# rlorenzo/facet

Measured on AMD Instinct MI355X. Metric: images/sec whole-node (TOPIQ+SAMP+CLIP+InsightFace ensemble), 1024² batch, higher is better.
Workload: dtype f32

## Files before the change

### facet_amd/csrc/engine.hip

```cpp
#include "engine.h"
#include "onnx_graph.h"
#include <algorithm>
#include <cmath>
#include <cstdlib>

namespace fe {

void WeightStore::set(const std::string& name, const float* data, const int64_t* shape, int ndim) {
  HostTensor h;
  h.shape.assign(shape, shape + ndim);
  h.data.assign(data, data + h.numel());
  t_[name] = std::move(h);
}
const HostTensor& WeightStore::get(const std::string& name) const {
  auto it = t_.find(name);
  if (it == t_.end()) throw Error("missing weight tensor '" + name + "'");
  return it->second;
}

float* DeviceWeights::upload(const std::vector<float>& v) {
  void* p = nullptr;
  const size_t b = v.size() * sizeof(float);
  FE_HIP(hipMalloc(&p, b ? b : 16));
  if (b) FE_HIP(hipMemcpy(p, v.data(), b, hipMemcpyHostToDevice));
  ptrs_.push_back(p);
  bytes_ += b;
  return (float*)p;
}
void* DeviceWeights::upload_raw(const void* data, size_t bytes) {
  void* p = nullptr;
  FE_HIP(hipMalloc(&p, bytes ? bytes : 16));
  if (bytes) FE_HIP(hipMemcpy(p, data, bytes, hipMemcpyHostToDevice));
  ptrs_.push_back(p);
  bytes_ += bytes;
  return p;
}
void DeviceWeights::release() {
  for (void* p : ptrs_) (void)hipFree(p);
  ptrs_.clear();
  bytes_ = 0;
}

const float* to_f32(Ctx& c, const bf16* p, size_t n) {
  float* f = c.arena.array<float>(n);
  launch_convert(p, f, n, c.stream);
  return f;
}
const float* to_f32(Ctx& c, const f16* p, size_t n) {
  float* f = c.arena.array<float>(n);
  launch_convert(p, f, n, c.stream);
  return f;
}

Ctx::~Ctx() {
  topiq.reset();
  for (auto& kv : resize_box_cache) { (void)hipFree(kv.second.kk); (void)hipFree(kv.second.bounds); }
  for (auto& kv : jpeg_cache) (void)hipFree(kv.second);
  if (jpegdec_stage) (void)hipHostFree(jpegdec_stage);
  arena.release();
  if (stream) (void)hipStreamDestroy(stream);
}

ConvW pack_conv(DeviceWeights& dw, const HostTensor& w, const std::vector<float>* scale, const std::vector<float>* shift) {
  FE_CHECK(w.shape.size() == 4 || w.shape.size() == 2, "conv weight rank %zu", w.shape.size());
  ConvW c;
  c.Cout = (int)w.shape[0];
  c.Cin = (int)w.shape[1];
  c.KH = w.shape.size() == 4 ? (int)w.shape[2] : 1;
  c.KW = w.shape.size() == 4 ? (int)w.shape[3] : 1;
  c.CinPad = (c.Cin + 3) & ~3;
  c.K = c.KH * c.KW * c.CinPad;
  c.Kp = (c.K + CONV_KALIGN - 1) / CONV_KALIGN * CONV_KALIGN;
  std::vector<float> packed((size_t)c.Cout * c.Kp, 0.f);
  const bool blocked = (c.CinPad % 16 == 0);
  const int ntaps = c.KH * c.KW;
  for (int co = 0; co < c.Cout; ++co)
    for (int ci = 0; ci < c.Cin; ++ci)
      for (int kh = 0; kh < c.KH; ++kh)
        for (int kw = 0; kw < c.KW; ++kw) {
          const int tap = kh * c.KW + kw;
          const size_t k = blocked ? ((size_t)(ci / 16) * ntaps + tap) * 16 + (ci % 16) : (size_t)tap * c.CinPad + ci;
          packed[(size_t)co * c.Kp + k] = w.data[(((size_t)co * c.Cin + ci) * c.KH + kh) * c.KW + kw];
        }
  const bool skip_f32 = dw.half_only && dw.prec != PREC_F32 && (c.KH * c.KW == 1 || ((c.Cin + 7) & ~7) % 16 == 0);
  if (!skip_f32) c.w = dw.upload(packed);
  if (!skip_f32 && c.Cout <= 2 && c.KH * c.KW > 1 && c.CinPad % 16 == 0) {
    const int T = c.KH * c.KW * c.Cout;
    c.KpT = (c.CinPad + CONV_KALIGN - 1) / CONV_KALIGN * CONV_KALIGN;
    std::vector<float> tp((size_t)T * c.KpT, 0.f);
    for (int t = 0; t < c.KH * c.KW; ++t)
      for (int co = 0; co < c.Cout; ++co)
        for (int ci = 0; ci < c.Cin; ++ci)
          tp[(size_t)(t * c.Cout + co) * c.KpT + ci] = w.data[(((size_t)co * c.Cin + ci) * c.KH + t / c.KW) * c.KW + t % c.KW];
    c.wtap = dw.upload(tp);
  }
  if (c.CinPad == 4 && c.KH == c.KW && (c.KH == 7 || c.KH == 3) && (c.Cout == 32 || c.Cout == 64)) {
    bool ch3_zero = true;
    const int taps = c.KH * c.KW, taps2 = (taps + 1) & ~1;
    for (int co = 0; co < c.Cout && c.Cin == 4; ++co)
      for (int t = 0; t < taps; ++t) ch3_zero = ch3_zero && w.data[((size_t)co * c.Cin + 3) * taps + t] == 0.f;
    if (ch3_zero) {
      std::vector<float> st((size_t)taps2 * c.Cout * 4, 0.f);
      for (int co = 0; co < c.Cout; ++co)
        for (int ci = 0; ci < c.Cin && ci < 3; ++ci)
          for (int t = 0; t < taps; ++t) st[((size_t)t * c.Cout + co) * 4 + ci] = w.data[((size_t)co * c.Cin + ci) * taps + t];
      c.wstem = dw.upload(st);
    }
  }
  static const int wino_min_cin = getenv("FE_WINO_MIN_CIN") ? atoi(getenv("FE_WINO_MIN_CIN")) : 96;
  static const int wino_form = getenv("FE_WINO_FORM") ? atoi(getenv("FE_WINO_FORM")) : 4;
  if (!skip_f32 && dw.prec == PREC_F32 && (wino_form == 2 || wino_form == 4) && c.KH == 3 && c.KW == 3 && c.Cin == c.CinPad && c.Cin % 32 == 0 && c.Cin >= wino_min_cin && c.Cout % 4 == 0) {
    static const double G2[4][3] = {{1, 0, 0}, {0.5, 0.5, 0.5}, {0.5, -0.5, 0.5}, {0, 0, 1}};
    static const double G4[6][3] = {{0.25, 0, 0}, {-1.0 / 6, -1.0 / 6, -1.0 / 6}, {-1.0 / 6, 1.0 / 6, -1.0 / 6},
                                    {1.0 / 24, 1.0 / 12, 1.0 / 6}, {1.0 / 24, -1.0 / 12, 1.0 / 6}, {0, 0, 1}};
    const int R = wino_form == 2 ? 4 : 6;
    auto Gm = [&](int a, int q) { return wino_form == 2 ? G2[a][q] : G4[a][q]; };
    std::vector<float> U((size_t)R * R * c.Cout * c.Cin);
    for (int co = 0; co < c.Cout; ++co)
      for (int ci = 0; ci < c.Cin; ++ci) {
        const float* g = &w.data[((size_t)co * c.Cin + ci) * 9];
        double tmp[6][3];
        for (int a = 0; a < R; ++a)
          for (int q = 0; q < 3; ++q) tmp[a][q] = Gm(a, 0) * g[q] + Gm(a, 1) * g[3 + q] + Gm(a, 2) * g[6 + q];
        for (int a = 0; a < R; ++a)
          for (int b = 0; b < R; ++b) {
            const double u = tmp[a][0] * Gm(b, 0) + tmp[a][1] * Gm(b, 1) + tmp[a][2] * Gm(b, 2);
            U[((size_t)(R * a + b) * c.Cout + co) * c.Cin + ci] = (float)u;
          }
      }
    c.wino = dw.upload(U);
    c.wino_m = wino_form;
  }
  if (scale) c.scale = dw.upload(*scale);
  if (shift) c.shift = dw.upload(*shift);
  if (dw.prec != PREC_F32) pack_conv_bf16(dw, w, c);
  return c;
}

void pack_conv_bf16(DeviceWeights& dw, const HostTensor& w, ConvW& c) {
  const int ntaps = c.KH * c.KW;
  c.CinPadH = (c.Cin + 7) & ~7;
  if (ntaps > 1) {
    if (c.CinPadH % 32 == 0) c.cb = 32;
    else if (c.CinPadH % 16 == 0) c.cb = 16;
    else return;
    if (ntaps >= 64) return;
  } else {
    c.cb = 32;
  }
  const int K = ntaps * c.CinPadH;
  c.KpH = (K + CONV_KALIGN_H - 1) / CONV_KALIGN_H * CONV_KALIGN_H;
  std::vector<uint16_t> packed((size_t)c.Cout * c.KpH, 0);
  for (int co = 0; co < c.Cout; ++co)
    for (int ci = 0; ci < c.Cin; ++ci)
      for (int t = 0; t < ntaps; ++t) {
        const size_t k = ntaps > 1 ? ((size_t)(ci / c.cb) * ntaps + t) * c.cb + (ci % c.cb) : (size_t)ci;
        packed[(size_t)co * c.KpH + k] = f32_to_half_bits(w.data[((size_t)co * c.Cin + ci) * ntaps + t], dw.prec);
      }
  c.wh = dw.upload_raw(packed.data(), packed.size() * sizeof(uint16_t));
  c.hprec = dw.prec;
  if (c.Cout <= 2 && ntaps > 1) {
    const int T = ntaps * c.Cout, T8 = (T + 7) & ~7;
    c.KpTH = (c.CinPadH + CONV_KALIGN_H - 1) / CONV_KALIGN_H * CONV_KALIGN_H;
    std::vector<uint16_t> tp((size_t)T8 * c.KpTH, 0);
    for (int t = 0; t < ntaps; ++t)
      for (int co = 0; co < c.Cout; ++co)
        for (int ci = 0; ci < c.Cin; ++ci)
          tp[(size_t)(t * c.Cout + co) * c.KpTH + ci] = f32_to_half_bits(w.data[((size_t)co * c.Cin + ci) * ntaps + t], dw.prec);
    c.wtap_h = dw.upload_raw(tp.data(), tp.size() * sizeof(uint16_t));
  }
}

ConvW build_conv(DeviceWeights& dw, const WeightStore& ws, const std::string& conv_prefix,
                 const std::string& bn_prefix, bool conv_bias, float bn_eps) {
  const HostTensor& w = ws.get(conv_prefix + ".weight");
  const int cout = (int)w.shape[0];
  std::vector<float> scale, shift;
  const bool bn = !bn_prefix.empty();
  if (bn) {
    const auto& g = ws.get(bn_prefix + ".weight").data;
    const auto& b = ws.get(bn_prefix + ".bias").data;
    const auto& mu = ws.get(bn_prefix + ".running_mean").data;
    const auto& var = ws.get(bn_prefix + ".running_var").data;
    FE_CHECK((int)g.size() == cout && (int)var.size() == cout, "bn %s size mismatch", bn_prefix.c_str());
    scale.resize(cout); shift.resize(cout);
    for (int i = 0; i < cout; ++i) {
      const float inv = 1.0f / std::sqrt(var[i] + bn_eps);
      scale[i] = g[i] * inv;
      float sh = b[i] - mu[i] * scale[i];
      if (conv_bias) sh += ws.get(conv_prefix + ".bias").data[i] * scale[i];
      shift[i] = sh;
    }
  } else if (conv_bias) {
    shift = ws.get(conv_prefix + ".bias").data;
    FE_CHECK((int)shift.size() == cout, "bias %s size mismatch", conv_prefix.c_str());
  }
  return pack_conv(dw, w, scale.empty() ? nullptr : &scale, shift.empty() ? nullptr : &shift);
}

ConvW build_linear(DeviceWeights& dw, const WeightStore& ws, const std::string& prefix, bool bias) {
  const HostTensor& w = ws.get(prefix + ".weight");
  FE_CHECK(w.shape.size() == 2, "linear %s weight rank", prefix.c_str());
  if (bias) {
    const auto& b = ws.get(prefix + ".bias").data;
    return pack_conv(dw, w, nullptr, &b);
  }
  return pack_conv(dw, w, nullptr, nullptr);
}

ConvW build_linear_rows(DeviceWeights& dw, const HostTensor& w, const HostTensor* b, int row0, int rows) {
  FE_CHECK(w.shape.size() == 2 && row0 + rows <= w.shape[0], "linear_rows: bad range");
  HostTensor sub;
  const int in = (int)w.shape[1];
  sub.shape = {rows, in};
// ... 22 lines not shown
  p.x = x.p; p.ldx = x.ld;
  p.w = w.w; p.scale = w.scale; p.shift = w.shift; p.slope = w.slope;
  FE_CHECK(o.act != ACT_PRELU || w.slope, "conv: PReLU without slopes");
  if (o.res) {
    FE_CHECK(o.res->c == y.c && o.res->pixels() == y.pixels(), "conv: residual shape mismatch");
    p.res = o.res->p; p.ldr = o.res->ld;
  }
  if (o.gate) {
    FE_CHECK(o.gate->pixels() == y.pixels() && (o.gate->c == 1 || o.gate->c == y.c), "conv: gate shape mismatch");
    p.gate = o.gate->p; p.ldg = o.gate->ld; p.gate_c1 = o.gate->c == 1;
  }
  p.y = y.p; p.ldy = y.ld;
  p.N = x.n; p.H = x.h; p.W = x.w; p.Cin = w.CinPad;
  p.Ho = y.h; p.Wo = y.w; p.Cout = w.Cout;
  p.KH = w.KH; p.KW = w.KW; p.sh = o.sh; p.sw = o.sw; p.ph = o.ph; p.pw = o.pw; p.dh = o.dh; p.dw = o.dw;
  FE_CHECK(y.h == conv_out_dim(x.h, w.KH, o.sh, o.ph, o.dh) && y.w == conv_out_dim(x.w, w.KW, o.sw, o.pw, o.dw),
           "conv: output dims %dx%d inconsistent with input %dx%d", y.h, y.w, x.h, x.w);
  p.K = w.K; p.Kp = w.Kp;
  p.M = (int)y.pixels();
  FE_CHECK(y.pixels() < (1ull << 31), "conv: M too large");
  p.act = o.act; p.res_after_act = o.res_after_act;
  p.variant = c.force_variant;
  if (w.wtap && o.act != ACT_PRELU && o.sh == 1 && o.sw == 1 && !o.res && !o.gate && p.variant == 0 && y.h == x.h && y.w == x.w) {
    const int T = w.KH * w.KW * w.Cout, Tp = (T + 3) & ~3;
    const size_t mark = c.arena.mark();
    Tensor z = c.arena.tensor(x.n, x.h, x.w, Tp);
    ConvParams q{};
    q.x = x.p; q.ldx = x.ld; q.w = w.wtap; q.y = z.p; q.ldy = Tp;
    q.N = x.n; q.H = x.h; q.W = x.w; q.Cin = w.CinPad; q.Ho = x.h; q.Wo = x.w; q.Cout = T;
    q.KH = q.KW = 1; q.sh = q.sw = q.dh = q.dw = 1;
    q.K = w.CinPad; q.Kp = w.KpT; q.M = (int)x.pixels();
    launch_conv(q, c.stream);
    launch_tap_gather(z.p, Tp, x.n, x.h, x.w, w.KH, w.KW, o.ph, o.pw, o.dh, o.dw, w.Cout, w.scale, w.shift, o.act, y.p,
                      y.ld, y.h, y.w, c.stream);
    c.arena.rewind(mark);
    c.flops_accum += 2.0 * p.M * (double)(w.KH * w.KW * w.Cin) * (w.CoutAlg ? w.CoutAlg : p.Cout);
    return;
  }
  static const bool no_wino = getenv("FE_NO_WINO") != nullptr;
  const bool wino_plain = !o.res && (o.act == ACT_NONE || o.act == ACT_RELU);
  if (w.wino && !no_wino && p.variant == 0 && o.sh == 1 && o.sw == 1 && o.ph == 1 && o.pw == 1 && o.dh == 1 && o.dw == 1 &&
      !o.gate && (wino_plain || (w.wino_m == 4 && (o.act == ACT_NONE || o.act == ACT_RELU || o.act == ACT_PRELU))) && y.h == x.h && y.w == x.w && (((uintptr_t)x.p | (uintptr_t)y.p) & 15) == 0 &&
      x.ld % 4 == 0 && y.ld % 4 == 0) {
    const int ts = w.wino_m, planes = (ts + 2) * (ts + 2);
    const int th = (x.h + ts - 1) / ts, tw = (x.w + ts - 1) / ts;
    const size_t tiles = (size_t)x.n * th * tw;
    const size_t wino_bytes = (size_t)planes * tiles * ((size_t)w.CinPad + w.Cout) * sizeof(float) + 1024;
    if (tiles < (1u << 30) / 36 && c.arena.mark() + wino_bytes <= c.arena.capacity()) {
      const size_t mark = c.arena.mark();
      float* V = (float*)c.arena.alloc((size_t)planes * tiles * w.CinPad * sizeof(float));
      float* Mb = (float*)c.arena.alloc((size_t)planes * tiles * w.Cout * sizeof(float));
      hipEvent_t e0 = nullptr, e1 = nullptr;
      if (c.profile) {
        FE_HIP(hipEventCreate(&e0)); FE_HIP(hipEventCreate(&e1));
        FE_HIP(hipEventRecord(e0, c.stream));
      }
      if (ts == 2) launch_wino_input(x, th, tw, V, c.stream);
      else launch_wino4_input(x, th, tw, V, c.stream);
      ConvParams g{};
      g.x = V; g.ldx = w.CinPad; g.w = w.wino; g.ldw = w.CinPad; g.y = Mb; g.ldy = w.Cout;
      g.M = (int)tiles; g.K = w.CinPad; g.Cout = w.Cout;
      g.N = 1; g.H = 1; g.W = g.M; g.Ho = 1; g.Wo = g.M; g.KH = g.KW = 1; g.sh = g.sw = g.dh = g.dw = 1;
      g.Kp = w.CinPad; g.Cin = w.CinPad;
      g.batch = planes; g.nb1 = 1; g.xs2 = (long long)tiles * w.CinPad; g.ws2 = (long long)w.Cout * w.CinPad; g.ys2 = (long long)tiles * w.Cout;
      launch_conv(g, c.stream);
      if (ts == 2) launch_wino_output(Mb, y, th, tw, w.scale, w.shift, o.act == ACT_RELU, c.stream);
      else launch_wino4_output(Mb, y, th, tw, w.scale, w.shift, o.act, w.slope, o.res, o.res_after_act, c.stream);
      if (c.profile) {
        FE_HIP(hipEventRecord(e1, c.stream));
        FE_HIP(hipEventSynchronize(e1));
        float ms = 0.f;
        FE_HIP(hipEventElapsedTime(&ms, e0, e1));
        (void)hipEventDestroy(e0); (void)hipEventDestroy(e1);
        char nm[128];
        snprintf(nm, sizeof nm, "wino3x3 M=%d K=%d N=%d", p.M, p.K, p.Cout);
        c.timings.push_back({nm, 2.0 * p.M * (double)(9 * w.Cin) * p.Cout, 0.0, ms});
      }
      c.arena.rewind(mark);
      c.flops_accum += 2.0 * p.M * (double)(w.KH * w.KW * w.Cin) * (w.CoutAlg ? w.CoutAlg : p.Cout);
      c.flops_saved += 2.0 * p.M * (double)(9 * w.Cin) * (w.CoutAlg ? w.CoutAlg : p.Cout) - 2.0 * (double)planes * (double)tiles * w.CinPad * w.Cout;
      return;
    }
  }
  static const bool no_splitk = getenv("FE_NO_SPLITK") != nullptr;
  if (!no_splitk && w.KH == 1 && w.KW == 1 && o.sh == 1 && o.sw == 1 && o.ph == 0 && o.pw == 0 && !o.gate && p.variant == 0 && p.M <= 256 &&
      w.CinPad >= (getenv("FE_SPLITK_MIN") ? atoi(getenv("FE_SPLITK_MIN")) : 2048) && w.K == w.CinPad &&
      (o.act == ACT_NONE || o.act == ACT_RELU || o.act == ACT_PRELU)) {
    int splits = 0;
    for (int s = 64; s >= 2; --s)
      if (w.CinPad % s == 0 && (w.CinPad / s) % 32 == 0 && w.CinPad / s >= 256) { splits = s; break; }
    const size_t part_bytes = (size_t)splits * p.M * w.Cout * sizeof(float);
    if (splits && c.arena.mark() + part_bytes + 1024 <= c.arena.capacity()) {
      const size_t mark = c.arena.mark();
      float* part = (float*)c.arena.alloc(part_bytes);
      const int Ks = w.CinPad / splits;
      hipEvent_t e0 = nullptr, e1 = nullptr;
      if (c.profile) {
        FE_HIP(hipEventCreate(&e0)); FE_HIP(hipEventCreate(&e1));
        FE_HIP(hipEventRecord(e0, c.stream));
      }
      ConvParams g{};
      g.x = x.p; g.ldx = x.ld; g.w = w.w; g.ldw = w.Kp; g.y = part; g.ldy = w.Cout;
      g.M = p.M; g.K = Ks; g.Kp = Ks; g.Cin = Ks; g.Cout = w.Cout;
      g.N = 1; g.H = 1; g.W = g.M; g.Ho = 1; g.Wo = g.M; g.KH = g.KW = 1; g.sh = g.sw = g.dh = g.dw = 1;
      g.batch = splits; g.nb1 = 1; g.xs2 = Ks; g.ws2 = Ks; g.ys2 = (long long)p.M * w.Cout;
      launch_conv(g, c.stream);
      launch_splitk_reduce(part, splits, p.M, w.Cout, w.scale, w.shift, w.slope, o.act, o.res ? o.res->p : nullptr, o.res ? o.res->ld : 0,
                           o.res_after_act, y.p, y.ld, c.stream);
      if (c.profile) {
        FE_HIP(hipEventRecord(e1, c.stream));
        FE_HIP(hipEventSynchronize(e1));
        float ms = 0.f;
        FE_HIP(hipEventElapsedTime(&ms, e0, e1));
        (void)hipEventDestroy(e0); (void)hipEventDestroy(e1);
        char nm[128];
        snprintf(nm, sizeof nm, "splitk%d 1x1 M=%d K=%d N=%d", splits, p.M, p.K, p.Cout);
        c.timings.push_back({nm, 2.0 * p.M * (double)w.Cin * (w.CoutAlg ? w.CoutAlg : p.Cout), 0.0, ms});
      }
      c.arena.rewind(mark);
      c.flops_accum += 2.0 * p.M * (double)w.Cin * (w.CoutAlg ? w.CoutAlg : p.Cout);
      return;
    }
  }
  static const bool no_stem = getenv("FE_NO_STEM") != nullptr;
  const bool stem = w.wstem && !no_stem && p.variant == 0 && o.sh == o.sw && o.ph == w.KH / 2 && o.pw == w.KW / 2 && o.dh == 1 && o.dw == 1 && !o.res &&
                    !o.gate && (o.act == ACT_NONE || o.act == ACT_RELU || o.act == ACT_PRELU);
  auto launch = [&]() {
    if (stem && launch_stem(x.p, x.ld, x.n, x.h, x.w, w.wstem, w.scale, w.shift, w.slope, w.Cout, w.KH, o.sh,
                            o.act == ACT_RELU ? 1 : (o.act == ACT_PRELU ? 2 : 0), y.p, y.ld, y.h, y.w, c.stream))
      return;
    launch_conv(p, c.stream);
  };
  if (c.profile) {
    hipEvent_t e0, e1;
    FE_HIP(hipEventCreate(&e0)); FE_HIP(hipEventCreate(&e1));
    FE_HIP(hipEventRecord(e0, c.stream));
    launch();
    FE_HIP(hipEventRecord(e1, c.stream));
    FE_HIP(hipEventSynchronize(e1));
    float ms = 0.f;
    FE_HIP(hipEventElapsedTime(&ms, e0, e1));
    (void)hipEventDestroy(e0); (void)hipEventDestroy(e1);
    char nm[128];
    snprintf(nm, sizeof nm, "conv%dx%d s%d d%d M=%d K=%d N=%d", w.KH, w.KW, o.sh, o.dh, p.M, p.K, p.Cout);
    double bytes = 4.0 * ((double)x.pixels() * x.c + (double)y.pixels() * y.c * (o.res ? 2 : 1) + (double)w.Cout * w.K);
    c.timings.push_back({nm, 2.0 * p.M * (double)(w.KH * w.KW * w.Cin) * (w.CoutAlg ? w.CoutAlg : p.Cout), bytes, ms});
  } else {
    launch();
  }
  c.flops_accum += 2.0 * p.M * (double)(w.KH * w.KW * w.Cin) * (w.CoutAlg ? w.CoutAlg : p.Cout);
}

template <class E>
static void conv_forward_half(Ctx& c, const ConvW& w, const TensorT<E>& x, const TensorT<E>& y, const ConvOptsT<E>& o) {
  if (!w.wh && w.w && PrecOf<E>::value != PREC_F32 && !o.res && !o.gate && x.ld == x.c && y.ld == y.c && x.c >= w.CinPad) {
    const size_t mark = c.arena.mark();
    Tensor xf = c.arena.tensor(x.n, x.h, x.w, x.c), yf = c.arena.tensor(y.n, y.h, y.w, y.c);
    launch_convert(x.p, xf.p, x.numel(), c.stream);
    ConvOpts of; of.sh = o.sh; of.sw = o.sw; of.ph = o.ph; of.pw = o.pw; of.dh = o.dh; of.dw = o.dw; of.act = o.act;
    conv_forward(c, w, xf.slice(0, w.CinPad), yf, of);
    launch_convert(yf.p, y.p, y.numel(), c.stream);
    c.arena.rewind(mark);
    return;
  }
  FE_CHECK(w.wh && w.hprec == PrecOf<E>::value, "conv(2-byte): this layer has no weights of the activations' type (model committed under another "
           "precision, or a 3-channel first layer)");
  FE_CHECK(x.c == w.CinPadH, "conv(bf16): input channels %d != packed Cin %d", x.c, w.CinPadH);
  FE_CHECK(y.c == w.Cout && y.n == x.n, "conv(bf16): output view mismatch (c=%d Cout=%d)", y.c, w.Cout);
  FE_CHECK(y.p || o.y32, "conv(2-byte): no output tensor");
// ... 448 lines not shown
```

### facet_amd/csrc/fe_common.h

```cpp
#pragma once
#include <hip/hip_runtime.h>
#include "fe_check.h"
#include <cstdint>
#include <cstdio>
#include <atomic>
#include <cstring>
#include <map>
#include <mutex>
#include <stdexcept>
#include <string>
#include <vector>

namespace fe {


#define FE_HIP(expr)                                                                      \
  do {                                                                                    \
    hipError_t _e = (expr);                                                               \
    if (_e != hipSuccess) {                                                               \
      char _b[512];                                                                       \
      snprintf(_b, sizeof _b, "%s:%d: %s -> %s", __FILE__, __LINE__, #expr,               \
               hipGetErrorString(_e));                                                    \
      throw fe::Error(_b);                                                                \
    }                                                                                     \
// ... 141 lines not shown
    FE_HIP(hipMalloc(&base_, bytes));
    cap_ = bytes;
    off_ = 0;
  }
  void release() {
    if (base_) (void)hipFree(base_);
    base_ = nullptr;
    cap_ = off_ = 0;
  }
  ~Arena() { release(); }
  void reset() { off_ = 0; }
  size_t mark() const { return off_; }
  void rewind(size_t m) { off_ = m; }
  size_t capacity() const { return cap_; }
  size_t high_water() const { return high_; }
  void* alloc(size_t bytes) {
    size_t a = (off_ + 255) & ~(size_t)255;
    FE_CHECK(a + bytes <= cap_, "arena exhausted: need %zu at %zu of %zu", bytes, a, cap_);
    off_ = a + bytes;
    if (off_ > high_) high_ = off_;
    return (char*)base_ + a;
  }
  template <class T>
  TensorT<T> tensor_t(int n, int h, int w, int c) {
    TensorT<T> t;
    t.n = n; t.h = h; t.w = w; t.c = c; t.ld = c;
    t.p = (T*)alloc(t.numel() * sizeof(T));
    return t;
  }
  Tensor tensor(int n, int h, int w, int c) { return tensor_t<float>(n, h, w, c); }
  template <class T>
  T* array(size_t count) { return (T*)alloc(count * sizeof(T)); }
 private:
  void* base_ = nullptr;
  size_t cap_ = 0, off_ = 0, high_ = 0;
};

template <class T>
struct ConvParamsT {
  const T* x; int ldx;
  const T* w;
  const float* scale;
  const float* shift;
  const float* slope;
  const T* res; int ldr;
  const T* gate; int ldg;
  T* y; int ldy;
  int N, H, W, Cin, Ho, Wo, Cout;
  int KH, KW, sh, sw, ph, pw, dh, dw;
  int K, Kp, M;
  int act;
  int res_after_act;
  int gate_c1;
  int vec_epi;
  int unit_stride;
  int ldw;
  int batch, nb1;
  long long xs1, xs2, ws1, ws2, ys1, ys2, hs1;
  int buf_ok; unsigned x_span, w_span;
  unsigned y_span, r_span, g_span;
  int variant;
  int cb;
  int pad_store;
  const float* res32; int ldr32;
  float* y32; int ldy32;
  unsigned r32_span, y32_span;
  int a_wrap;
  int split_lo_off;
  int exact_act;
};
using ConvParams = ConvParamsT<float>;
using ConvParamsH = ConvParamsT<bf16>;

struct ConvW {
  float* w = nullptr;
  float* scale = nullptr;
  float* shift = nullptr;
  float* slope = nullptr;
  int Cout = 0, Cin = 0, CinPad = 0, KH = 1, KW = 1, K = 0, Kp = 0;
  int CoutAlg = 0;
  float* wtap = nullptr;
  int wino_m = 0;
  float* wino = nullptr;
  float* wstem = nullptr;
  float* wn16 = nullptr;
  int KpT = 0;
  void* wh = nullptr;
  int hprec = 0;
  int KpH = 0, cb = 0, CinPadH = 0;
  void* wtap_h = nullptr;
  int KpTH = 0;
  uint8_t* w8 = nullptr;
  float* w8_scale = nullptr;
};

template <class T>
struct ConvOptsT {
  int sh = 1, sw = 1, ph = 0, pw = 0, dh = 1, dw = 1;
  int act = ACT_NONE;
  const TensorT<T>* res = nullptr;
  int res_after_act = 0;
  const TensorT<T>* gate = nullptr;
  const TensorT<float>* res32 = nullptr;
  const TensorT<float>* y32 = nullptr;
};
using ConvOpts = ConvOptsT<float>;

constexpr int CONV_KALIGN = 32;
constexpr int CONV_KALIGN_H = 64;

void launch_conv(const ConvParams& p, hipStream_t s);
void launch_wino_input(const Tensor& x, int th, int tw, float* V, hipStream_t s);
void launch_wino_output(const float* Mb, const Tensor& y, int th, int tw, const float* scale, const float* shift, int relu, hipStream_t s);
void launch_wino4_input(const Tensor& x, int th, int tw, float* V, hipStream_t s);
void launch_wino4_output(const float* Mb, const Tensor& y, int th, int tw, const float* scale, const float* shift, int act, const float* slope,
                         const Tensor* res, int res_after_act, hipStream_t s);
template <class TO>
bool launch_stem(const float* x, int ldx, int N, int H, int W, const float* wstem, const float* scale, const float* shift, const float* slope,
                 int Cout, int k, int stride, int act, TO* y, int ldy, int Ho, int Wo, hipStream_t s);
void launch_conv_narrow(const ConvParams& p, hipStream_t s);
void launch_conv_dma(const ConvParams& p, int tile, hipStream_t s);
void launch_conv_bf16(const ConvParamsH& p, hipStream_t s);
void launch_conv_bf16(const ConvParamsT<f16>& p, hipStream_t s);
template <class T, class Launch>
inline bool conv_split_by_images(const ConvParamsT<T>& p, Launch&& launch) {
  if (p.batch > 1 || p.N <= 1 || (long long)p.N * p.Ho * p.Wo != (long long)p.M) return false;
  const unsigned long long in_img = (unsigned long long)p.H * p.W * p.ldx * sizeof(T);
  unsigned long long out_img = (unsigned long long)p.Ho * p.Wo * (unsigned long long)(p.ldy > p.ldr ? p.ldy : p.ldr) * sizeof(T);
  const unsigned long long out32_img = (unsigned long long)p.Ho * p.Wo * (unsigned long long)(p.ldy32 > p.ldr32 ? p.ldy32 : p.ldr32) * sizeof(float);
  if ((p.y32 || p.res32) && out32_img > out_img) out_img = out32_img;
  const unsigned long long per_img = in_img > out_img ? in_img : out_img;
  constexpr unsigned long long LIMIT = 0xF0000000ull;
  if (per_img >= LIMIT) return false;
  const int ng = (int)(LIMIT / per_img);
  if (ng >= p.N) return false;
  for (int i0 = 0; i0 < p.N; i0 += ng) {
    ConvParamsT<T> q = p;
    const int n = ng < p.N - i0 ? ng : p.N - i0;
    const size_t opix = (size_t)i0 * p.Ho * p.Wo;
    q.N = n; q.M = n * p.Ho * p.Wo;
    q.x = p.x + (size_t)i0 * p.H * p.W * p.ldx;
    if (p.y) q.y = p.y + opix * p.ldy;
    if (p.y32) q.y32 = p.y32 + opix * p.ldy32;
    if (p.res32) q.res32 = p.res32 + opix * p.ldr32;
    if (p.res) q.res = p.res + opix * p.ldr;
    if (p.gate) q.gate = p.gate + opix * p.ldg;
    launch(q);
  }
  return true;
}

double conv_flops(const ConvParams& p);

void launch_u8_to_nhwc4_norm(const uint8_t* src, float* dst, size_t pixels, const float mean[3],
                             const float stdv[3], int bgr, hipStream_t s);
template <class T> void launch_nchw_to_nhwc(const float* src, T* dst, int n, int c, int h, int w, int cpad, hipStream_t s);
template <class T> void launch_nhwc_to_nchw(const T* src, int lds_, float* dst, int n, int c, int h, int w, hipStream_t s);
template <class T> void launch_maxpool(const TensorT<T>& x, const TensorT<T>& y, int k, int stride, int pad, hipStream_t s);
template <class T> void launch_bilinear(const TensorT<T>& x, const TensorT<T>& y, hipStream_t s);
template <class T> void launch_adaptive_avgpool(const TensorT<T>& x, const TensorT<T>& y, hipStream_t s);
void launch_convert(const float* x, bf16* y, size_t n, hipStream_t s);
void launch_convert(const bf16* x, float* y, size_t n, hipStream_t s);
void launch_convert(const float* x, f16* y, size_t n, hipStream_t s);
void launch_convert(const f16* x, float* y, size_t n, hipStream_t s);
void launch_splitk_reduce(const float* part, int splits, int M, int N, const float* scale, const float* shift, const float* slope, int act,
                          const float* res, int ldr, int res_after_act, float* y, int ldy, hipStream_t s);
template <class T>
void launch_tap_gather(const T* z, int ldz, int n, int h, int w, int kh, int kw, int ph, int pw, int dh, int dw,
                       int cout, const float* scale, const float* shift, int act, T* y, int ldy, int ho, int wo,
                       hipStream_t s);
void launch_attention(const float* q, int ldq, const float* k, int ldk, const float* vt, int lp, const float* bv, float* o,
                      int ldo, int B, int H, int Lq, int Lk, int dmodel, int causal, hipStream_t s);
void launch_attention(const bf16* q, int ldq, const bf16* k, int ldk, const bf16* vt, int lp, const float* bv, bf16* o,
                      int ldo, int B, int H, int Lq, int Lk, int dmodel, int causal, hipStream_t s);
void launch_attention(const f16* q, int ldq, const f16* k, int ldk, const f16* vt, int lp, const float* bv, f16* o,
                      int ldo, int B, int H, int Lq, int Lk, int dmodel, int causal, hipStream_t s);
void launch_attention_split(const f16* q, const f16* k, int ld, int lo_off, const f16* vt_hi, const f16* vt_lo, int lp, f16* o, int ldo, int o_lo_off,
                            int B, int H, int Lq, int Lk, int dmodel, hipStream_t s);
template <class TI, class TW, class TO>
void launch_gemm_skinny(const TI* x, int ldx, const TW* w, int ldw, const float* scale, const float* shift, TO* y,
                        int ldy, int M, int N, int K, int act, hipStream_t s);
void launch_sigmoid(const Tensor& x, const Tensor& y, hipStream_t s);
void launch_add(const Tensor& a, const Tensor& b, const Tensor& y, hipStream_t s);
void launch_layernorm_split(const float* x, int ldx, f16* y, int ldy, const float* g, const float* b, int rows, int d, float eps, hipStream_t s);
void launch_split_hi_lo(const float* x, f16* y, size_t rows, int cols, hipStream_t s);
template <class T, class TO>
void launch_layernorm(const T* x, int ldx, TO* y, int ldy, const float* g, const float* b,
                      int rows, int d, float eps, hipStream_t s);
void launch_softmax_rows(float* x, int ld, int rows, int d, hipStream_t s);
void launch_softmax_rows_pad(float* x, int ld, int rows, int d, hipStream_t s);
template <class T>
void launch_add_rows_bcast(T* y, int ldy, const float* pos, int rows, int L, int d, hipStream_t s);

void launch_affine_act(const Tensor& x, const Tensor& y, const float* scale, const float* shift, int act, const float* slope,
                       hipStream_t s);
void launch_binary(const Tensor& a, const Tensor& b, const Tensor& y, int op, int act, hipStream_t s);
void launch_gather_strided(const float* src, float* dst, const long long dims[6], const long long sstr[6], hipStream_t s);
void launch_nearest(const Tensor& x, const Tensor& y, hipStream_t s);
void launch_avgpool(const Tensor& x, const Tensor& y, int k, int stride, int pad, int include_pad, hipStream_t s);
// ... 49 lines not shown
```

Baseline: 231.4.

## Add fused Winograd F(2x2,3x3) MFMA kernel for 64-channel 3x3 convs

Adds a single-kernel Winograd F(2,3) path for stride-1, pad-1 3x3 convolutions with 56-64 input and 33-64 output channels. It stages input patches through double-buffered LDS, does the input transform in registers, runs the per-plane products on 32x32x2 f32 MFMA, and applies the output transform, affine, activation and residual in the epilogue. This replaces the separate input-transform, GEMM and output-transform launches and their intermediate buffers. It also restricts split-K for 1x1 convs to small tile grids and caches the split-K threshold environment variable. The added cost is a new, complex kernel with one block per CU and a 2x2 Winograd form that saves less arithmetic than F(4,3).

```diff
diff --git a/facet_amd/csrc/engine.hip b/facet_amd/csrc/engine.hip
--- a/facet_amd/csrc/engine.hip
+++ b/facet_amd/csrc/engine.hip
@@ -1,5 +1,6 @@
 #include "engine.h"
 #include "onnx_graph.h"
+#include "wino64_maps.h"
 #include <algorithm>
 #include <cmath>
 #include <cstdlib>
@@ -130,6 +131,11 @@
       }
     c.wino = dw.upload(U);
     c.wino_m = wino_form;
+  }
+  if (!skip_f32 && dw.prec == PREC_F32 && c.KH == 3 && c.KW == 3 && c.CinPad >= 56 && c.CinPad <= 64 && c.Cout > 32 && c.Cout <= 64 && c.Cout % 4 == 0) {
+    std::vector<float> U(w64::U_FLOATS);
+    w64::pack_u(w.data.data(), c.Cout, c.Cin, U.data());
+    c.wino64 = dw.upload(U);
   }
   if (scale) c.scale = dw.upload(*scale);
   if (shift) c.shift = dw.upload(*shift);
@@ -318,9 +324,37 @@
       return;
     }
   }
+  static const bool no_wino64 = getenv("FE_NO_WINO64") != nullptr;
+  if (w.wino64 && !no_wino64 && p.variant == 0 && (o.act == ACT_NONE || o.act == ACT_RELU || o.act == ACT_PRELU) && o.sh == 1 && o.sw == 1 && o.ph == 1 && o.pw == 1 && o.dh == 1 && o.dw == 1 && !o.gate && y.h == x.h &&
+      y.w == x.w && (((uintptr_t)x.p | (uintptr_t)y.p | (uintptr_t)(o.res ? o.res->p : nullptr)) & 15) == 0 && x.ld % 4 == 0 && y.ld % 4 == 0 &&
+      (!o.res || o.res->ld % 4 == 0) && (unsigned long long)x.h * x.w * x.ld * 4ull < 0xF0000000ull) {
+    hipEvent_t e0 = nullptr, e1 = nullptr;
+    if (c.profile) {
+      FE_HIP(hipEventCreate(&e0)); FE_HIP(hipEventCreate(&e1));
+      FE_HIP(hipEventRecord(e0, c.stream));
+    }
+    launch_wino64(x, y, w.wino64, w.scale, w.shift, w.slope, o.act, o.res, o.res_after_act, c.stream);
+    const double direct = 2.0 * p.M * (double)(9 * w.Cin) * (w.CoutAlg ? w.CoutAlg : p.Cout);
+    if (c.profile) {
+      FE_HIP(hipEventRecord(e1, c.stream));
+      FE_HIP(hipEventSynchronize(e1));
+      float ms = 0.f;
+      FE_HIP(hipEventElapsedTime(&ms, e0, e1));
+      (void)hipEventDestroy(e0); (void)hipEventDestroy(e1);
+      char nm[128];
+      snprintf(nm, sizeof nm, "wino64 3x3 M=%d K=%d N=%d", p.M, p.K, p.Cout);
+      const double bytes = 4.0 * ((double)x.pixels() * x.c + (double)y.pixels() * y.c * (o.res ? 2 : 1) + (double)w64::U_FLOATS);
+      c.timings.push_back({nm, direct, bytes, ms});
+    }
+    const double tiles = (double)x.n * ((x.h + 1) / 2) * ((x.w + 1) / 2);
+    c.flops_accum += direct;
+    c.flops_saved += direct - 2.0 * 16.0 * tiles * 64.0 * w.Cout;
+    return;
+  }
   static const bool no_splitk = getenv("FE_NO_SPLITK") != nullptr;
+  static const int splitk_min = getenv("FE_SPLITK_MIN") ? atoi(getenv("FE_SPLITK_MIN")) : 2048;
   if (!no_splitk && w.KH == 1 && w.KW == 1 && o.sh == 1 && o.sw == 1 && o.ph == 0 && o.pw == 0 && !o.gate && p.variant == 0 && p.M <= 256 &&
-      w.CinPad >= (getenv("FE_SPLITK_MIN") ? atoi(getenv("FE_SPLITK_MIN")) : 2048) && w.K == w.CinPad &&
+      w.CinPad >= splitk_min && w.K == w.CinPad && (size_t)((p.M + 127) / 128) * ((w.Cout + 63) / 64) < 64 &&
       (o.act == ACT_NONE || o.act == ACT_RELU || o.act == ACT_PRELU)) {
     int splits = 0;
     for (int s = 64; s >= 2; --s)
diff --git a/facet_amd/csrc/fe_common.h b/facet_amd/csrc/fe_common.h
--- a/facet_amd/csrc/fe_common.h
+++ b/facet_amd/csrc/fe_common.h
@@ -247,6 +247,7 @@
   float* wtap = nullptr;
   int wino_m = 0;
   float* wino = nullptr;
+  float* wino64 = nullptr;
   float* wstem = nullptr;
   float* wn16 = nullptr;
   int KpT = 0;
@@ -280,6 +281,8 @@
 void launch_wino4_input(const Tensor& x, int th, int tw, float* V, hipStream_t s);
 void launch_wino4_output(const float* Mb, const Tensor& y, int th, int tw, const float* scale, const float* shift, int act, const float* slope,
                          const Tensor* res, int res_after_act, hipStream_t s);
+void launch_wino64(const Tensor& x, const Tensor& y, const float* U, const float* scale, const float* shift, const float* slope, int act,
+                   const Tensor* res, int res_after_act, hipStream_t s);
 template <class TO>
 bool launch_stem(const float* x, int ldx, int N, int H, int W, const float* wstem, const float* scale, const float* shift, const float* slope,
                  int Cout, int k, int stride, int act, TO* y, int ldy, int Ho, int Wo, hipStream_t s);
diff --git a/facet_amd/csrc/kernels_wino64.hip b/facet_amd/csrc/kernels_wino64.hip
--- /dev/null
+++ b/facet_amd/csrc/kernels_wino64.hip
@@ -0,0 +1,205 @@
+#include "fe_common.h"
+#include "wino64_maps.h"
+
+namespace fe {
+
+struct W64Params {
+  const float* x; int ldx, cin;
+  int N, H, W;
+  float* y; int ldy, cout;
+  const float* U;
+  const float *scale, *shift, *slope;
+  const float* res; int ldr;
+  int res_after_act;
+  int bx, by, nblocks;
+};
+
+constexpr int W64_PATCH_FLOATS = w64::CHUNK_UNITS * 2;
+
+template <int A>
+__global__ __launch_bounds__(256, 1) __attribute__((amdgpu_waves_per_eu(1, 1))) void wino64_kernel(const W64Params p) {
+  using namespace w64;
+  __shared__ __attribute__((aligned(16))) float sP[2 * W64_PATCH_FLOATS];
+  const int t = threadIdx.x, lane = t & 63, wave = __builtin_amdgcn_readfirstlane(t >> 6);
+  const int tg = wave & 1, half = wave >> 1;
+  const int tl = lane & 31, kk = lane >> 5;
+  const int ty = tile_y(tg, tl), tx = tile_x(tl);
+  constexpr int act = A;
+
+  int pc_py[PIECES_PER_THREAD], pc_px[PIECES_PER_THREAD], pc_dst[PIECES_PER_THREAD];
+#pragma unroll
+  for (int i = 0; i < PIECES_PER_THREAD; ++i) {
+    const int idx = t + 256 * i, pixel = idx / PARTS, part = idx % PARTS;
+    pc_py[i] = pixel / PATCH; pc_px[i] = pixel - pc_py[i] * PATCH;
+    pc_dst[i] = idx < PIECES ? 2 * patch_unit(2 * part, pc_py[i], pc_px[i]) : -1;
+  }
+  const int part4 = (t % PARTS) * 4;
+  auto block_origin = [&](const int v, int& b, int& y0, int& x0) {
+    const int per = p.bx * p.by;
+    b = v / per;
+    const int rem = v - b * per, byi = rem / p.bx;
+    y0 = byi * BLOCK; x0 = (rem - byi * p.bx) * BLOCK;
+  };
+  fe_v4f pf[PIECES_PER_THREAD];
+  typedef unsigned w64_v4u __attribute__((ext_vector_type(4)));
+  constexpr unsigned OOB = 0xFFFFFFF0u;
+  const unsigned img_bytes = (unsigned)p.H * (unsigned)p.W * (unsigned)p.ldx * 4u;
+  auto fetch_stage = [&](const int v, const int c) __attribute__((always_inline)) {
+    const bool live = v < p.nblocks;
+    int b, y0, x0;
+    block_origin(live ? v : 0, b, y0, x0);
+    const __amdgpu_buffer_rsrc_t rs = __builtin_amdgcn_make_buffer_rsrc(const_cast<float*>(p.x + (size_t)b * p.H * p.W * p.ldx), 0, (int)img_bytes, 0x00020000);
+    const bool ch_in = live && c * CHUNK_CH + part4 < p.cin;
+#pragma unroll
+    for (int i = 0; i < PIECES_PER_THREAD; ++i) {
+      const int gy = y0 - 1 + pc_py[i], gx = x0 - 1 + pc_px[i];
+      const bool in = pc_dst[i] >= 0 && ch_in && (unsigned)gy < (unsigned)p.H && (unsigned)gx < (unsigned)p.W;
+      const unsigned off = in ? ((unsigned)(gy * p.W + gx) * (unsigned)p.ldx + (unsigned)(c * CHUNK_CH + part4)) * 4u : OOB;
+      pf[i] = __builtin_bit_cast(fe_v4f, (w64_v4u)__builtin_amdgcn_raw_buffer_load_b128(rs, (int)off, 0, 0));
+    }
+  };
+  auto store_stage = [&](const int buf) __attribute__((always_inline)) {
+    float* const pd = sP + buf * W64_PATCH_FLOATS;
+#pragma unroll
+    for (int i = 0; i < PIECES_PER_THREAD; ++i)
+      if (pc_dst[i] >= 0) {
+        *reinterpret_cast<float2*>(pd + pc_dst[i]) = make_float2(pf[i].x, pf[i].y);
+        *reinterpret_cast<float2*>(pd + pc_dst[i] + 2 * PAIR_UNITS) = make_float2(pf[i].z, pf[i].w);
+      }
+  };
+
+  const float* const ubase = p.U + u_index(0, half, 0, lane, 0);
+  fe_v4f ua[STEPS_PER_CHUNK][4];
+  auto fetch_u = [&](const int step, fe_v4f (&u)[4]) __attribute__((always_inline)) {
+#pragma unroll
+    for (int q = 0; q < 4; ++q) u[q] = *reinterpret_cast<const fe_v4f*>(ubase + step * U_STEP_FLOATS + q * 256);
+  };
+#pragma unroll
+  for (int s0 = 0; s0 < STEPS_PER_CHUNK; ++s0) fetch_u(s0, ua[s0]);
+  fetch_stage(blockIdx.x, 0);
+  store_stage(0);
+  __syncthreads();
+
+  const int lane_unit = patch_unit(kk, 2 * ty, 2 * tx);
+  for (int v = blockIdx.x; v < p.nblocks; v += gridDim.x) {
+    fe_f32x16 acc[16];
+#pragma unroll
+    for (int pl = 0; pl < 16; ++pl)
+#pragma unroll
+      for (int e = 0; e < 16; ++e) acc[pl][e] = 0.f;
+
+#pragma unroll 1
+    for (int c = 0; c < NCHUNK; ++c) {
+      if (c + 1 < NCHUNK) fetch_stage(v, c + 1);
+      else fetch_stage(v + (int)gridDim.x, 0);
+      const float* const buf = sP + (c & 1) * W64_PATCH_FLOATS + 2 * lane_unit;
+      float2 dq[2][16];
+      auto read_pair = [&](const int j, float2 (&d)[16]) __attribute__((always_inline)) {
+#pragma unroll
+        for (int dy = 0; dy < 4; ++dy)
+#pragma unroll
+          for (int dx = 0; dx < 4; ++dx)
+            d[4 * dy + dx] = *reinterpret_cast<const float2*>(buf + 2 * (2 * j * PAIR_UNITS + dy * ROW_UNITS + (dx & 1) * (ROW_UNITS / 2) + (dx >> 1)));
+      };
+      const int nstage = ((c + 1) & (NCHUNK - 1)) * STEPS_PER_CHUNK;
+      read_pair(0, dq[0]);
+#pragma unroll
+      for (int j = 0; j < STEPS_PER_CHUNK / 2; ++j) {
+        if (j + 1 < STEPS_PER_CHUNK / 2) read_pair(j + 1, dq[(j + 1) & 1]);
+        __builtin_amdgcn_sched_barrier(0);
+#pragma unroll
+        for (int s2 = 0; s2 < 2; ++s2) {
+          float d[16], vv[16];
+#pragma unroll
+          for (int i = 0; i < 16; ++i) d[i] = s2 ? dq[j & 1][i].y : dq[j & 1][i].x;
+          input_transform(d, vv);
+#pragma unroll
+          for (int pl = 0; pl < 16; ++pl) acc[pl] = __builtin_amdgcn_mfma_f32_32x32x2f32(ua[2 * j + s2][pl >> 2][pl & 3], vv[pl], acc[pl], 0, 0, 0);
+          __builtin_amdgcn_sched_barrier(0);
+          fetch_u(nstage + 2 * j + s2, ua[2 * j + s2]);
+        }
+      }
+      store_stage((c + 1) & 1);
+      __syncthreads();
+    }
+
+    int b, y0, x0;
+    block_origin(v, b, y0, x0);
+    const int oy = y0 + 2 * ty, ox = x0 + 2 * tx;
+    size_t pix[4]; bool ok[4];
+#pragma unroll
+    for (int i = 0; i < 4; ++i) {
+      const int yy = oy + (i >> 1), xx = ox + (i & 1);
+      ok[i] = yy < p.H && xx < p.W;
+      pix[i] = ok[i] ? ((size_t)b * p.H + yy) * p.W + xx : 0;
+    }
+    float4 scv[4], sfv[4], slv[4];
+#pragma unroll
+    for (int g = 0; g < 4; ++g) {
+      const int cb = acc_channel(half, lane, 4 * g), cl = cb < p.cout ? cb : 0;
+      scv[g] = p.scale ? *reinterpret_cast<const float4*>(p.scale + cl) : make_float4(1.f, 1.f, 1.f, 1.f);
+      sfv[g] = p.shift ? *reinterpret_cast<const float4*>(p.shift + cl) : make_float4(0.f, 0.f, 0.f, 0.f);
+      slv[g] = act == ACT_PRELU ? *reinterpret_cast<const float4*>(p.slope + cl) : make_float4(0.f, 0.f, 0.f, 0.f);
+    }
+#pragma unroll
+    for (int g = 0; g < 4; ++g) {
+      const int cb = acc_channel(half, lane, 4 * g);
+      if (cb >= p.cout) continue;
+      float o[4][4];
+#pragma unroll
+      for (int e = 0; e < 4; ++e) {
+        float m[16], yq[4];
+#pragma unroll
+        for (int pl = 0; pl < 16; ++pl) m[pl] = acc[pl][4 * g + e];
+        output_transform(m, yq);
+#pragma unroll
+        for (int i = 0; i < 4; ++i) o[i][e] = yq[i];
+      }
+      const float4 sc = scv[g], sf = sfv[g], sl = slv[g];
+#pragma unroll
+      for (int i = 0; i < 4; ++i) {
+        if (!ok[i]) continue;
+        float4 r = make_float4(0.f, 0.f, 0.f, 0.f);
+        if (p.res) r = *reinterpret_cast<const float4*>(p.res + pix[i] * p.ldr + cb);
+        float4 q;
+        q.x = o[i][0] * sc.x + sf.x; q.y = o[i][1] * sc.y + sf.y; q.z = o[i][2] * sc.z + sf.z; q.w = o[i][3] * sc.w + sf.w;
+        if (p.res && !p.res_after_act) { q.x += r.x; q.y += r.y; q.z += r.z; q.w += r.w; }
+        if (act == ACT_PRELU) {
+          q.x = q.x > 0.f ? q.x : q.x * sl.x; q.y = q.y > 0.f ? q.y : q.y * sl.y;
+          q.z = q.z > 0.f ? q.z : q.z * sl.z; q.w = q.w > 0.f ? q.w : q.w * sl.w;
+        } else {
+          q.x = fe_apply_act(q.x, act); q.y = fe_apply_act(q.y, act); q.z = fe_apply_act(q.z, act); q.w = fe_apply_act(q.w, act);
+        }
+        if (p.res && p.res_after_act) { q.x += r.x; q.y += r.y; q.z += r.z; q.w += r.w; }
+        *reinterpret_cast<float4*>(p.y + pix[i] * p.ldy + cb) = q;
+      }
+    }
+  }
+}
+
+void launch_wino64(const Tensor& x, const Tensor& y, const float* U, const float* scale, const float* shift, const float* slope, int act,
+                   const Tensor* res, int res_after_act, hipStream_t s) {
+  FE_CHECK(x.c > 0 && x.c <= 64 && x.c % 4 == 0 && y.c > 0 && y.c <= 64 && y.c % 4 == 0 && y.n == x.n && y.h == x.h && y.w == x.w, "wino64: %dx%dx%d -> %dx%dx%d", x.h,
+           x.w, x.c, y.h, y.w, y.c);
+  FE_CHECK(x.ld % 4 == 0 && y.ld % 4 == 0 && (((uintptr_t)x.p | (uintptr_t)y.p | (uintptr_t)U) & 15) == 0, "wino64: operands must be 16-byte aligned");
+  FE_CHECK(!res || (res->ld % 4 == 0 && ((uintptr_t)res->p & 15) == 0 && res->c == y.c && res->pixels() == y.pixels()), "wino64: residual view");
+  FE_CHECK(act == ACT_NONE || act == ACT_RELU || (act == ACT_PRELU && slope), "wino64: activation %d (PReLU needs slopes)", act);
+  FE_CHECK((unsigned long long)x.h * x.w * x.ld * 4ull < 0xF0000000ull, "wino64: one image must stay below 4 GiB (32-bit buffer offsets)");
+  W64Params p{};
+  p.x = x.p; p.ldx = x.ld; p.cin = x.c; p.N = x.n; p.H = x.h; p.W = x.w;
+  p.y = y.p; p.ldy = y.ld; p.cout = y.c;
+  p.U = U; p.scale = scale; p.shift = shift; p.slope = slope;
+  p.res = res ? res->p : nullptr; p.ldr = res ? res->ld : 0;
+  p.res_after_act = res_after_act;
+  p.bx = (x.w + w64::BLOCK - 1) / w64::BLOCK; p.by = (x.h + w64::BLOCK - 1) / w64::BLOCK;
+  const long long nb = (long long)x.n * p.bx * p.by;
+  FE_CHECK(nb < (1ll << 30), "wino64: too many blocks");
+  p.nblocks = (int)nb;
+  const int grid = p.nblocks < 256 ? p.nblocks : 256;
+  if (act == ACT_NONE) hipLaunchKernelGGL(wino64_kernel<ACT_NONE>, dim3(grid), dim3(256), 0, s, p);
+  else if (act == ACT_RELU) hipLaunchKernelGGL(wino64_kernel<ACT_RELU>, dim3(grid), dim3(256), 0, s, p);
+  else hipLaunchKernelGGL(wino64_kernel<ACT_PRELU>, dim3(grid), dim3(256), 0, s, p);
+  FE_HIP(hipGetLastError());
+}
+
+}
diff --git a/facet_amd/csrc/wino64_maps.h b/facet_amd/csrc/wino64_maps.h
--- /dev/null
+++ b/facet_amd/csrc/wino64_maps.h
@@ -0,0 +1,82 @@
+#pragma once
+
+#if defined(__HIPCC__)
+#define W64_HD __host__ __device__ __forceinline__
+#else
+#define W64_HD inline
+#endif
+
+namespace fe {
+namespace w64 {
+
+constexpr int BLOCK = 16;
+constexpr int PATCH = BLOCK + 2;
+constexpr int CHUNK_CH = 8;
+constexpr int NCHUNK = 64 / CHUNK_CH;
+constexpr int STEPS_PER_CHUNK = CHUNK_CH / 2;
+constexpr int NSTEPS = NCHUNK * STEPS_PER_CHUNK;
+constexpr int ROW_UNITS = 20;
+constexpr int PAIR_UNITS = PATCH * ROW_UNITS;
+constexpr int CHUNK_UNITS = (CHUNK_CH / 2) * PAIR_UNITS;
+constexpr int PARTS = CHUNK_CH / 4;
+constexpr int PIECES = PATCH * PATCH * PARTS;
+constexpr int PIECES_PER_THREAD = (PIECES + 255) / 256;
+constexpr int U_STEP_FLOATS = 2 * 4 * 64 * 4;
+constexpr int U_FLOATS = NSTEPS * U_STEP_FLOATS;
+
+W64_HD int tile_y(int tg, int tl) { return 4 * tg + (tl >> 3); }
+W64_HD int tile_x(int tl) { return tl & 7; }
+W64_HD int channel(int step, int k) { return 4 * (step >> 1) + 2 * k + (step & 1); }
+W64_HD int acc_channel(int half, int lane, int e) { return half * 32 + 8 * (e >> 2) + 4 * (lane >> 5) + (e & 3); }
+W64_HD int u_index(int step, int half, int q, int lane, int j) { return ((((step * 2 + half) * 4 + q) * 64 + lane) << 2) + j; }
+W64_HD int patch_unit(int pair, int py, int px) { return pair * PAIR_UNITS + py * ROW_UNITS + (px & 1) * (ROW_UNITS / 2) + (px >> 1); }
+
+W64_HD void input_transform(const float d[16], float v[16]) {
+  float t[16];
+  for (int c = 0; c < 4; ++c) {
+    t[0 + c] = d[0 + c] - d[8 + c];
+    t[4 + c] = d[4 + c] + d[8 + c];
+    t[8 + c] = d[8 + c] - d[4 + c];
+    t[12 + c] = d[4 + c] - d[12 + c];
+  }
+  for (int a = 0; a < 4; ++a) {
+    v[4 * a + 0] = t[4 * a + 0] - t[4 * a + 2];
+    v[4 * a + 1] = t[4 * a + 1] + t[4 * a + 2];
+    v[4 * a + 2] = t[4 * a + 2] - t[4 * a + 1];
+    v[4 * a + 3] = t[4 * a + 1] - t[4 * a + 3];
+  }
+}
+W64_HD void output_transform(const float m[16], float y[4]) {
+  float s[8];
+  for (int b = 0; b < 4; ++b) {
+    s[b] = (m[b] + m[4 + b]) + m[8 + b];
+    s[4 + b] = (m[4 + b] - m[8 + b]) - m[12 + b];
+  }
+  for (int i = 0; i < 2; ++i) {
+    y[2 * i + 0] = (s[4 * i + 0] + s[4 * i + 1]) + s[4 * i + 2];
+    y[2 * i + 1] = (s[4 * i + 1] - s[4 * i + 2]) - s[4 * i + 3];
+  }
+}
+
+inline void pack_u(const float* w, int Cout, int Cin, float* U) {
+  static const double G[4][3] = {{1, 0, 0}, {0.5, 0.5, 0.5}, {0.5, -0.5, 0.5}, {0, 0, 1}};
+  for (int i = 0; i < U_FLOATS; ++i) U[i] = 0.f;
+  for (int step = 0; step < NSTEPS; ++step)
+    for (int half = 0; half < 2; ++half)
+      for (int lane = 0; lane < 64; ++lane) {
+        const int co = half * 32 + (lane & 31), ci = channel(step, lane >> 5);
+        if (co >= Cout || ci >= Cin) continue;
+        const float* g = w + ((long long)co * Cin + ci) * 9;
+        double tmp[4][3];
+        for (int a = 0; a < 4; ++a)
+          for (int q = 0; q < 3; ++q) tmp[a][q] = G[a][0] * g[q] + G[a][1] * g[3 + q] + G[a][2] * g[6 + q];
+        for (int a = 0; a < 4; ++a)
+          for (int b = 0; b < 4; ++b) {
+            const double u = tmp[a][0] * G[b][0] + tmp[a][1] * G[b][1] + tmp[a][2] * G[b][2];
+            U[u_index(step, half, a, lane, b)] = (float)u;
+          }
+      }
+}
+
+}
+}
```

New measurement: 234.3 (median of 6 runs). 1.01x the previous value.
